# ZhonghuaYi/EI-Nexus_official

Hardware: AMD Instinct MI355X
Metric: event-image pairs/s (extract+match, 346x260, 1024 kpts) (higher is better)
Workload: dtype f32; 1 GPU; B32 346x260 5-bin event voxel + gray image, VGG(event)+SuperPoint(image) extractors, MNN matcher, k=1024; global_batch=32, event_bins=5, parallelism=dp1 (pairs sharded, metric all-reduce only), log_assignment=False, dense_outputs=False, same_scene_pairs=False, weights=seeded synthetic, descriptor-head bias calibrated (per-channel mean removed)

## Files before the change

ei-nexus_official_amd/csrc/detect.hip:

```cpp
#include <algorithm>

#include "einx_common.h"

namespace {

__device__ __forceinline__ bool mask_on(const uint8_t* mask, int b, int H, int W, int h0, int w0, int Hp, int Wp, int y, int x,
                                        int dilate, int replicate) {
  const int r = dilate ? 1 : 0;
  bool any = false;
#pragma unroll
  for (int dy = -1; dy <= 1; ++dy)
#pragma unroll
    for (int dx = -1; dx <= 1; ++dx) {
      const int yy = y + dy, xx = x + dx, sy = yy - h0, sx = xx - w0;
      const bool ok = dy >= -r && dy <= r && dx >= -r && dx <= r && yy >= 0 && yy < Hp && xx >= 0 && xx < Wp &&
                      (replicate || (sy >= 0 && sy < H && sx >= 0 && sx < W));
      const uint8_t m = mask[((size_t)b * H + min(max(sy, 0), H - 1)) * W + min(max(sx, 0), W - 1)];
      any |= ok && m != 0;
    }
  return any;
}

__global__ __launch_bounds__(256) void score65_kernel(const float* logits, int B, int hc, int wc, const uint8_t* mask, int H, int W,
                                                      int h0, int w0, int dilate, int replicate, int border, float* prob, float* score,
                                                      int32_t* zero_ptr, int zero_n, float* crop) {
  if ((int)(blockIdx.x * 256 + threadIdx.x) < zero_n) zero_ptr[blockIdx.x * 256 + threadIdx.x] = 0;
  const int cells = hc * wc;
  const int lane = threadIdx.x & 63, wave = threadIdx.x >> 6;
  const int j = lane & 7, i = lane >> 3;
  const int gid = (blockIdx.x * 4 + wave) * 8 + j;
  const bool valid = gid < B * cells;
  const int g = valid ? gid : B * cells - 1;
  const int b = g / cells, cell = g % cells;
  const int h = cell / wc, w = cell % wc;
  const float* l = logits + (size_t)b * 65 * cells + cell;
  float v[8];
#pragma unroll
  for (int k = 0; k < 8; ++k) v[k] = l[(size_t)(8 * i + k) * cells];
  const float v64 = l[(size_t)64 * cells];
  float mx = v64;
#pragma unroll
  for (int k = 0; k < 8; ++k) mx = fmaxf(mx, v[k]);
  mx = fmaxf(mx, __shfl_xor(mx, 8, 64));
  mx = fmaxf(mx, __shfl_xor(mx, 16, 64));
  mx = fmaxf(mx, __shfl_xor(mx, 32, 64));
  float e[8];
#pragma unroll
  for (int k = 0; k < 8; ++k) e[k] = einx_expf(v[k] - mx);
  const float e64 = einx_expf(v64 - mx);
  float s = 0.0f;
#pragma unroll
  for (int c = 0; c < 64; ++c) s = s + __shfl(e[c & 7], j + 8 * (c >> 3), 64);
  s = s + e64;
  if (!valid) return;
  const int Hp = hc * 8, Wp = wc * 8;
  float* pr = prob + (size_t)b * 65 * cells + cell;
  const int y = h * 8 + i;
  unsigned cols = 0x3ffu;
  if (mask) {
    cols = 0;
    const int r = dilate ? 1 : 0;
#pragma unroll
    for (int dy = -1; dy <= 1; ++dy) {
      const int yy = y + dy, sy = yy - h0;
      const bool rok = dy >= -r && dy <= r && yy >= 0 && yy < Hp && (replicate || (sy >= 0 && sy < H));
      const uint8_t* mrow = mask + ((size_t)b * H + min(max(sy, 0), H - 1)) * W;
      uint8_t m[10];
#pragma unroll
      for (int k = 0; k < 10; ++k) m[k] = mrow[min(max(w * 8 - 1 + k - w0, 0), W - 1)];
#pragma unroll
      for (int k = 0; k < 10; ++k) {
        const int xx = w * 8 - 1 + k, sx = xx - w0;
        if (rok && xx >= 0 && xx < Wp && (replicate || (sx >= 0 && sx < W)) && m[k]) cols |= 1u << k;
      }
    }
  }
  const unsigned window = (mask && !dilate) ? 2u : 7u;
  float out[8];
#pragma unroll
  for (int k = 0; k < 8; ++k) {
    const float p = e[k] / s;
    pr[(size_t)(8 * i + k) * cells] = p;
    const int x = w * 8 + k;
    float t = p;
    if (!((cols >> k) & window)) t = 0.0f;
    if (border > 0 && (y < border || y >= Hp - border || x < border || x >= Wp - border)) t = 0.0f;
    out[k] = t;
  }
  if (i == 0) pr[(size_t)64 * cells] = e64 / s;
  f32x4* dst = reinterpret_cast<f32x4*>(score + ((size_t)b * Hp + y) * Wp + w * 8);
  dst[0] = f32x4{out[0], out[1], out[2], out[3]};
  dst[1] = f32x4{out[4], out[5], out[6], out[7]};
  if (crop) {
    const int uy = y - h0;
    if (uy >= 0 && uy < H) {
      float* cr = crop + ((size_t)b * H + uy) * W - w0 + w * 8;
#pragma unroll
      for (int k = 0; k < 8; ++k) {
        const int ux = w * 8 + k - w0;
        if (ux >= 0 && ux < W) cr[k] = out[k];
      }
    }
  }
}

__global__ void score1_kernel(const float* logits, int B, int Hp, int Wp, const uint8_t* mask, int H, int W, int h0, int w0,
                              int dilate, int replicate, int border, float* prob, float* score, int32_t* zero_ptr, int zero_n,
                              float* crop) {
  const int n = Hp * Wp;
  const int gid = blockIdx.x * blockDim.x + threadIdx.x;
  if (gid < zero_n) zero_ptr[gid] = 0;
  if (gid >= B * n) return;
  const int b = gid / n, p = gid % n;
  const int y = p / Wp, x = p % Wp;
  float v = einx_sigmoidf(logits[gid]);
  if (mask && !mask_on(mask, b, H, W, h0, w0, Hp, Wp, y, x, dilate, replicate)) v = 0.0f;
  if (border > 0 && (y < border || y >= Hp - border || x < border || x >= Wp - border)) v = 0.0f;
  prob[gid] = v;
  score[gid] = v;
  if (crop) {
    const int uy = y - h0, ux = x - w0;
    if (uy >= 0 && uy < H && ux >= 0 && ux < W) crop[((size_t)b * H + uy) * W + ux] = v;
  }
}

__global__ void dense_positions_kernel(const float* score, int B, int H, int W, int xy, float* out) {
  const size_t n = (size_t)B * H * W;
  const size_t gid = (size_t)blockIdx.x * blockDim.x + threadIdx.x;
  if (gid >= n) return;
  const int p = (int)(gid % ((size_t)H * W));
  const float fy = (float)(p / W) + 0.5f, fx = (float)(p % W) + 0.5f;
  float* o = out + gid * 3;
  o[0] = xy ? fx : fy;
  o[1] = xy ? fy : fx;
  o[2] = score[gid];
}

__global__ void border_kernel(float* score, int B, int Hp, int Wp, int border) {
  const int n = Hp * Wp;
  const int gid = blockIdx.x * blockDim.x + threadIdx.x;
  if (gid >= B * n) return;
  const int p = gid % n;
  const int y = p / Wp, x = p % Wp;
  if (y < border || y >= Hp - border || x < border || x >= Wp - border) score[gid] = 0.0f;
}

constexpr int NMS_TH = 32, NMS_TW = 64, NMS_MAXR = 4, NMS_THREADS = 512;

template <int R>
__global__ __launch_bounds__(NMS_THREADS) void nms_pass_kernel(const float* src, float* dst, int Hp, int Wp, int tilesX, int tilesY,
                                                       int32_t* flags, int it, int nIt) {
  constexpr int VH = NMS_TH + 4 * R, VW = NMS_TW + 4 * R;
  constexpr int MH = NMS_TH + 2 * R, MW = NMS_TW + 2 * R;
// ... 42 lines not shown
  for (int i = tid; i < MH * MW; i += NMS_THREADS) {
    const int my = i / MW, mx = i % MW;
    const int vy = my + R;
    const float* row = vals + vy * VW + mx;
    const float c = row[R];
    const int y = y0 - R + my, x = x0 - R + mx;
    float left = row[0], right = row[R + 1];
#pragma unroll
    for (int dx = 1; dx < R; ++dx) {
      left = fmaxf(left, row[dx]);
      right = fmaxf(right, row[R + 1 + dx]);
    }
    float above = r9[(vy - R) * MW + mx], below = r9[(vy + 1) * MW + mx];
#pragma unroll
    for (int dy = 1; dy < R; ++dy) {
      above = fmaxf(above, r9[(vy - R + dy) * MW + mx]);
      below = fmaxf(below, r9[(vy + 1 + dy) * MW + mx]);
    }
    const bool ok = y >= 0 && y < Hp && x >= 0 && x < Wp && left < c && above < c && right <= c && below <= c;
    ismax[i] = ok ? 1 : 0;
  }
  __syncthreads();
  for (int i = tid; i < MH * NMS_TW; i += NMS_THREADS) {
    const int my = i / NMS_TW, tx = i % NMS_TW;
    const uint8_t* row = ismax + my * MW + tx;
    unsigned o = 0;
#pragma unroll
    for (int dx = 0; dx <= 2 * R; ++dx) o |= row[dx];
    rowor[i] = (uint8_t)o;
  }
  __syncthreads();
  int my_changed = 0;
  for (int i = tid; i < NMS_TH * NMS_TW; i += NMS_THREADS) {
    const int ty = i / NMS_TW, tx = i % NMS_TW;
    const int y = y0 + ty, x = x0 + tx;
    if (y >= Hp || x >= Wp) continue;
    const float c = vals[(ty + 2 * R) * VW + tx + 2 * R];
    unsigned o = 0;
#pragma unroll
    for (int dy = 0; dy <= 2 * R; ++dy) o |= rowor[(ty + dy) * NMS_TW + tx];
    const bool sup = o != 0 && !ismax[(ty + R) * MW + tx + R];
    float out = c;
    if (c != 0.0f && sup) {
      out = 0.0f;
      my_changed = 1;
    }
    d[(size_t)y * Wp + x] = out;
  }
  if (my_changed) changed = 1;
  __syncthreads();
  if (tid == 0 && changed) atomicOr(&flags[b * nIt + it], 1);
}

struct __attribute__((aligned(16))) Nms4Smem {
  static constexpr int R = 4;
  static constexpr int VH = NMS_TH + 4 * R, VW = NMS_TW + 4 * R;
  static constexpr int MH = NMS_TH + 2 * R, MW = NMS_TW + 2 * R;
  static constexpr int G = MW / 8, TG = NMS_TW / 8;
  float vals[VH * VW];
  float r9[VH * MW];
  uint8_t rowok8[VH * G];
  uint8_t ismax8[MH * (G + 1)];
  uint8_t rowor8[MH * TG];
  int changed;
};

template <bool COHERENT>
__device__ __forceinline__ void nms4_tile(Nms4Smem& sm, const float* s, float* d, int Hp, int Wp, int y0, int x0) {
  constexpr int R = Nms4Smem::R, VH = Nms4Smem::VH, VW = Nms4Smem::VW, MH = Nms4Smem::MH, MW = Nms4Smem::MW, G = Nms4Smem::G, TG = Nms4Smem::TG;
  const int tid = threadIdx.x;
  constexpr int NLOAD = (VH * VW + NMS_THREADS - 1) / NMS_THREADS;
  float staged[NLOAD];
#pragma unroll
  for (int k = 0; k < NLOAD; ++k) {
    const int i = tid + k * NMS_THREADS;
    const int ii = i < VH * VW ? i : 0;
    const int y = y0 - 2 * R + ii / VW, x = x0 - 2 * R + ii % VW;
    const bool in = y >= 0 && y < Hp && x >= 0 && x < Wp;
    const float* src_p = s + (size_t)(in ? y : 0) * Wp + (in ? x : 0);
    const float v = COHERENT ? __hip_atomic_load(const_cast<float*>(src_p), __ATOMIC_RELAXED, __HIP_MEMORY_SCOPE_AGENT) : *src_p;
    staged[k] = in ? v : 0.0f;
  }
#pragma unroll
  for (int k = 0; k < NLOAD; ++k) {
    const int i = tid + k * NMS_THREADS;
    if (i < VH * VW) sm.vals[i] = staged[k];
  }
  __syncthreads();
  if (tid < VH * G) {
    const int vy = tid / G, g = tid % G;
    float v[16];
    const float* row = sm.vals + vy * VW + g * 8;
#pragma unroll
    for (int q = 0; q < 4; ++q) {
      const f32x4 t = *reinterpret_cast<const f32x4*>(row + 4 * q);
      v[4 * q] = t[0];
      v[4 * q + 1] = t[1];
      v[4 * q + 2] = t[2];
      v[4 * q + 3] = t[3];
    }
    float m9[8];
    unsigned ok = 0;
#pragma unroll
    for (int k = 0; k < 8; ++k) {
      float left = v[k], right = v[k + 5];
#pragma unroll
      for (int t = 1; t < 4; ++t) {
        left = fmaxf(left, v[k + t]);
        right = fmaxf(right, v[k + 5 + t]);
      }
      const float c = v[k + 4];
      m9[k] = fmaxf(fmaxf(left, right), c);
      ok |= (left < c && right <= c) ? (1u << k) : 0u;
    }
    float* o = sm.r9 + vy * MW + g * 8;
    *reinterpret_cast<f32x4*>(o) = f32x4{m9[0], m9[1], m9[2], m9[3]};
    *reinterpret_cast<f32x4*>(o + 4) = f32x4{m9[4], m9[5], m9[6], m9[7]};
    sm.rowok8[tid] = (uint8_t)ok;
  }
  __syncthreads();
  if (tid < MH * G) {
    const int my = tid / G, g = tid % G;
    const int vy = my + R;
    float above[8], below[8];
#pragma unroll
    for (int k = 0; k < 8; ++k) above[k] = below[k] = 0.0f;
#pragma unroll
    for (int dy = 1; dy <= R; ++dy) {
      const float* ra = sm.r9 + (vy - dy) * MW + g * 8;
      const float* rb = sm.r9 + (vy + dy) * MW + g * 8;
      const f32x4 a0 = *reinterpret_cast<const f32x4*>(ra), a1 = *reinterpret_cast<const f32x4*>(ra + 4);
      const f32x4 b0 = *reinterpret_cast<const f32x4*>(rb), b1 = *reinterpret_cast<const f32x4*>(rb + 4);
#pragma unroll
      for (int k = 0; k < 4; ++k) {
        above[k] = dy == 1 ? a0[k] : fmaxf(above[k], a0[k]);
        above[k + 4] = dy == 1 ? a1[k] : fmaxf(above[k + 4], a1[k]);
        below[k] = dy == 1 ? b0[k] : fmaxf(below[k], b0[k]);
        below[k + 4] = dy == 1 ? b1[k] : fmaxf(below[k + 4], b1[k]);
      }
    }
    const float* crow = sm.vals + vy * VW + g * 8 + R;
    const f32x4 c0 = *reinterpret_cast<const f32x4*>(crow), c1 = *reinterpret_cast<const f32x4*>(crow + 4);
    const unsigned rok = sm.rowok8[vy * G + g];
    const int y = y0 - R + my;
    unsigned bits = 0;
#pragma unroll
    for (int k = 0; k < 8; ++k) {
      const float c = k < 4 ? c0[k] : c1[k - 4];
      const int x = x0 - R + g * 8 + k;
      const bool okk = ((rok >> k) & 1u) && y >= 0 && y < Hp && x >= 0 && x < Wp && above[k] < c && below[k] <= c;
      bits |= okk ? (1u << k) : 0u;
    }
    sm.ismax8[my * (G + 1) + g] = (uint8_t)bits;
    if (g == 0) sm.ismax8[my * (G + 1) + G] = 0;
  }
  __syncthreads();
  if (tid < MH * TG) {
    const int my = tid / TG, t8 = tid % TG;
    const unsigned w = (unsigned)sm.ismax8[my * (G + 1) + t8] | ((unsigned)sm.ismax8[my * (G + 1) + t8 + 1] << 8) |
                       ((unsigned)sm.ismax8[my * (G + 1) + t8 + 2] << 16);
    unsigned r = 0;
#pragma unroll
    for (int dx = 0; dx <= 2 * R; ++dx) r |= w >> dx;
    sm.rowor8[tid] = (uint8_t)(r & 0xFFu);
  }
  __syncthreads();
  int my_changed = 0;
  if (tid < NMS_TH * TG) {
    const int ty = tid / TG, t8 = tid % TG;
    unsigned o8 = 0;
#pragma unroll
    for (int dy = 0; dy <= 2 * R; ++dy) o8 |= sm.rowor8[(ty + dy) * TG + t8];
    const unsigned iw = (unsigned)sm.ismax8[(ty + R) * (G + 1) + t8] | ((unsigned)sm.ismax8[(ty + R) * (G + 1) + t8 + 1] << 8);
    const unsigned is8 = (iw >> R) & 0xFFu;
    const unsigned sup = o8 & ~is8;
    const float* crow = sm.vals + (ty + 2 * R) * VW + t8 * 8 + 2 * R;
    const f32x4 c0 = *reinterpret_cast<const f32x4*>(crow), c1 = *reinterpret_cast<const f32x4*>(crow + 4);
    const int y = y0 + ty;
    if (y < Hp) {
      float out[8];
#pragma unroll
      for (int k = 0; k < 8; ++k) {
        const float c = k < 4 ? c0[k] : c1[k - 4];
        const bool kill = c != 0.0f && ((sup >> k) & 1u);
        out[k] = kill ? 0.0f : c;
        if (kill && x0 + t8 * 8 + k < Wp) my_changed = 1;
      }
      float* o = d + (size_t)y * Wp + x0 + t8 * 8;
      if (x0 + t8 * 8 + 7 < Wp && (Wp & 3) == 0) {
        *reinterpret_cast<f32x4*>(o) = f32x4{out[0], out[1], out[2], out[3]};
        *reinterpret_cast<f32x4*>(o + 4) = f32x4{out[4], out[5], out[6], out[7]};
      } else {
#pragma unroll
        for (int k = 0; k < 8; ++k)
          if (x0 + t8 * 8 + k < Wp) o[k] = out[k];
      }
    }
  }
  if (my_changed) sm.changed = 1;
}

__global__ __launch_bounds__(NMS_THREADS) void nms_pass4_kernel(const float* src, float* dst, int Hp, int Wp, int tilesX, int tilesY,
                                                                int32_t* flags, int it, int nIt) {
  __shared__ Nms4Smem sm;
  int bid = xcd_contiguous((int)blockIdx.x, (int)gridDim.x);
  const int txi = bid % tilesX;
  bid /= tilesX;
  const int tyi = bid % tilesY;
  const int b = bid / tilesY;
  if (it >= 2 && flags[b * nIt + it - 1] == 0) return;
  if (threadIdx.x == 0) sm.changed = 0;
  nms4_tile<false>(sm, src + (size_t)b * Hp * Wp, dst + (size_t)b * Hp * Wp, Hp, Wp, tyi * NMS_TH, txi * NMS_TW);
  __syncthreads();
  if (threadIdx.x == 0 && sm.changed) atomicOr(&flags[b * nIt + it], 1);
}

constexpr int NMS_FIN_MAXT = 2048;
constexpr int kNmsFinishMaxPasses = 256;
__global__ __launch_bounds__(NMS_THREADS) void nms4_finish_kernel(float* bufA, float* bufB, int Hp, int Wp, int tilesX, int tilesY,
                                                                  int32_t* flags, int nIt, int max_passes) {
  __shared__ Nms4Smem sm;
  __shared__ uint8_t dirty[2][NMS_FIN_MAXT];
  __shared__ int any_changed;
  const int b = blockIdx.x;
  if (flags[b * nIt + nIt - 1] == 0) return;
  const int tid = threadIdx.x;
  const int ntiles = tilesX * tilesY;
  const bool track = ntiles <= NMS_FIN_MAXT;
  float* src = bufA + (size_t)b * Hp * Wp;
  float* dst = bufB + (size_t)b * Hp * Wp;
  if (track)
    for (int i = tid; i < ntiles; i += NMS_THREADS) {
      dirty[0][i] = 1;
      dirty[1][i] = 0;
    }
  __syncthreads();
  int cur = 0;
  int left = 1;
  for (int pass = 0; pass < max_passes; ++pass) {
    if (tid == 0) any_changed = 0;
    for (int t = 0; t < ntiles; ++t) {
      const int txi = t % tilesX, tyi = t / tilesX;
      bool need = !track;
      if (track) {
        for (int dy = -1; dy <= 1 && !need; ++dy)
          for (int dx = -1; dx <= 1; ++dx) {
            const int yy = tyi + dy, xx = txi + dx;
            if (yy >= 0 && yy < tilesY && xx >= 0 && xx < tilesX && dirty[cur][yy * tilesX + xx]) need = true;
          }
      }
      if (!need) continue;
      if (tid == 0) sm.changed = 0;
      __syncthreads();
      nms4_tile<true>(sm, src, dst, Hp, Wp, tyi * NMS_TH, txi * NMS_TW);
      __syncthreads();
      if (tid == 0 && sm.changed) {
        any_changed = 1;
        if (track) dirty[cur ^ 1][t] = 1;
      }
      __syncthreads();
    }
    asm volatile("s_waitcnt vmcnt(0)" ::: "memory");
    __syncthreads();
    left = any_changed;
    if (track)
      for (int i = tid; i < ntiles; i += NMS_THREADS) dirty[cur][i] = 0;
    cur ^= 1;
    float* tmp = src;
    src = dst;
    dst = tmp;
    __syncthreads();
    if (!left) break;
  }
  if (tid == 0) flags[b * nIt + nIt - 1] = left ? 1 : 0;
}

constexpr int SEL_THREADS = 1024;

struct SelArgs {
  const float* map;
  const int32_t* flags;
  float* nms_out;
  float* positions;
  int32_t* indices;
  int32_t* counts;
  float* thr_out;
  int32_t* not_converged;
  int Hp, Wp, H, W, h0, w0;
  int top_k, lo, hi, cap, ordering_xy, nIt;
  float det_thr;
};

__device__ __forceinline__ int block_excl_scan(int v, int* total, int* scratch ) {
  const int lane = threadIdx.x & 63, wave = threadIdx.x >> 6;
  int incl = v;
#pragma unroll
  for (int off = 1; off < 64; off <<= 1) {
    const int t = __shfl_up(incl, off, 64);
    if (lane >= off) incl += t;
  }
  if (lane == 63) scratch[wave] = incl;
  __syncthreads();
  if (threadIdx.x == 0) {
    int run = 0;
    for (int w = 0; w < SEL_THREADS / 64; ++w) {
      const int t = scratch[w];
      scratch[w] = run;
// ... 328 lines not shown
    if (i < nz) {
      v = cval[i];
      fi = cidx[i];
      y = fi / a.Wp;
      x = fi % a.Wp;
      const int uy = y - a.h0, ux = x - a.w0;
      keep = v > thr && uy >= 0 && uy < a.H && ux >= 0 && ux < a.W;
    }
    int total;
    const int pos = base + block_excl_scan(keep ? 1 : 0, &total, scratch);
    if (keep && pos < a.cap) {
      const float py = ((float)y + 0.5f) - (float)a.h0, px = ((float)x + 0.5f) - (float)a.w0;
      float* o = a.positions + ((size_t)b * a.cap + pos) * 3;
      o[0] = a.ordering_xy ? px : py;
      o[1] = a.ordering_xy ? py : px;
      o[2] = v;
      a.indices[(size_t)b * a.cap + pos] = fi;
    }
    base += total;
  }
  if (tid == 0) a.counts[b] = base;
}

__global__ void nms_crop_kernel(const float* map, const float* thr, int B, int Hp, int Wp, int h0, int w0, int H, int W, float* out) {
  const size_t n = (size_t)B * H * W;
  const size_t gid = (size_t)blockIdx.x * blockDim.x + threadIdx.x;
  if (gid >= n) return;
  const int b = (int)(gid / ((size_t)H * W));
  const int r = (int)(gid % ((size_t)H * W));
  const float v = map[((size_t)b * Hp + (r / W + h0)) * Wp + r % W + w0];
  out[gid] = v > thr[b] ? v : 0.0f;
}

void topk_ranks(int N, int k, int* lo, int* hi) {
  const float q = (float)(N - k) / (float)N;
  const float rank = q * (float)(N - 1);
  *lo = (int)floorf(rank);
  *hi = (int)ceilf(rank);
}

}

EINX_EXPORT int einx_score_map(const float* logits, int B, int C, int hc, int wc, const uint8_t* mask, int H, int W, int h0, int w0,
                               int dilate, int border, float* prob, float* score, void* stream) {
  return einx_score_map_zero(logits, B, C, hc, wc, mask, H, W, h0, w0, dilate, EINX_MASK_PAD_ZERO, border, prob, score, nullptr, 0, nullptr,
                             stream);
}

EINX_EXPORT int einx_score_map_pad(const float* logits, int B, int C, int hc, int wc, const uint8_t* mask, int mask_pad, int H, int W, int h0,
                                   int w0, int dilate, int border, float* prob, float* score, void* stream) {
  return einx_score_map_zero(logits, B, C, hc, wc, mask, H, W, h0, w0, dilate, mask_pad, border, prob, score, nullptr, 0, nullptr, stream);
}

int einx_score_map_zero(const float* logits, int B, int C, int hc, int wc, const uint8_t* mask, int H, int W, int h0, int w0, int dilate,
                        int mask_pad, int border, float* prob, float* score, int32_t* zero_ptr, int zero_n, float* crop, void* stream) {
  EINX_CHECK_ARG(mask_pad == EINX_MASK_PAD_ZERO || mask_pad == EINX_MASK_PAD_REPLICATE, "mask_pad must be EINX_MASK_PAD_ZERO or EINX_MASK_PAD_REPLICATE");
  EINX_CHECK_ARG(!mask || (H > 0 && W > 0), "a mask needs the un-padded size");
  const int replicate = mask_pad == EINX_MASK_PAD_REPLICATE;
  EINX_CHECK_ARG(!crop || (H > 0 && W > 0), "the cropped map needs the un-padded size");
  EINX_CHECK_ARG(logits && prob && score, "null pointer");
  EINX_CHECK_ARG(zero_n == 0 || (zero_ptr && (long)zero_n <= (long)(C == 65 ? einx_cdiv(B * hc * wc, 32) : einx_cdiv(B * hc * wc, 256)) * 256),
                 "more words to zero than threads in the launch");
  EINX_CHECK_ARG(C == 65 || C == 1, "detector head must have 65 or 1 channels");
  EINX_CHECK_ARG(B > 0 && hc > 0 && wc > 0, "bad shape");
  hipStream_t s = (hipStream_t)stream;
  EINX_PROF("score_map (score65/score1)", s);
  if (C == 65) {
    const int n = B * hc * wc;
    hipLaunchKernelGGL(score65_kernel, dim3(einx_cdiv(n, 32)), dim3(256), 0, s, logits, B, hc, wc, mask, H, W, h0, w0, dilate, replicate, border,
                       prob, score, zero_ptr, zero_n, crop);
  } else {
    const int n = B * hc * wc;
    hipLaunchKernelGGL(score1_kernel, dim3(einx_cdiv(n, 256)), dim3(256), 0, s, logits, B, hc, wc, mask, H, W, h0, w0, dilate, replicate, border,
                       prob, score, zero_ptr, zero_n, crop);
  }
  EINX_CHECK_LAUNCH();
  return EINX_OK;
}

EINX_EXPORT int einx_remove_border(float* score, int B, int Hp, int Wp, int border, void* stream) {
  EINX_CHECK_ARG(score, "null pointer");
  if (border <= 0) return EINX_OK;
  const int n = B * Hp * Wp;
  hipLaunchKernelGGL(border_kernel, dim3(einx_cdiv(n, 256)), dim3(256), 0, (hipStream_t)stream, score, B, Hp, Wp, border);
  EINX_CHECK_LAUNCH();
  return EINX_OK;
}

EINX_EXPORT int einx_dense_positions(const float* score, int B, int H, int W, int ordering_xy, float* out, void* stream) {
  EINX_CHECK_ARG(score && out, "null pointer");
  EINX_CHECK_ARG(B > 0 && H > 0 && W > 0, "bad shape");
  const size_t n = (size_t)B * H * W;
  hipLaunchKernelGGL(dense_positions_kernel, dim3((unsigned)((n + 255) / 256)), dim3(256), 0, (hipStream_t)stream, score, B, H, W, ordering_xy, out);
  EINX_CHECK_LAUNCH();
  return EINX_OK;
}

EinxDetectWs einx_detect_carve(WsCarver& c, const einx_detect_params* p) {
  const size_t map = (size_t)p->B * p->Hp * p->Wp;
  const EinxDetectWs w{c.take<float>(map), c.take<float>(map), c.take<int32_t>((size_t)p->B * (p->nms_iters > 0 ? p->nms_iters : 1)),
                       p->radius > 0 ? p->B * p->nms_iters : 0};
  c.slack(256);
  return w;
}

EINX_EXPORT size_t einx_detect_ws_bytes(const einx_detect_params* p) {
  if (!p) return 0;
  WsCarver c{nullptr};
  einx_detect_carve(c, p);
  return c.bytes;
}

EINX_EXPORT int einx_detect(const float* score, const einx_detect_params* p, void* ws, float* nms_out, float* positions,
                            int32_t* indices, int32_t* counts, float* thr, int32_t* not_converged, void* stream) {
  return einx_detect_prezeroed(score, p, ws, nms_out, positions, indices, counts, thr, not_converged, 0, nullptr, stream);
}

int einx_detect_prezeroed(const float* score, const einx_detect_params* p, void* ws, float* nms_out, float* positions, int32_t* indices,
                          int32_t* counts, float* thr, int32_t* not_converged, int flags_zeroed, const float** final_map, void* stream) {
  EINX_CHECK_ARG(score && p && ws && positions && indices && counts && thr && not_converged, "null pointer");
  EINX_CHECK_ARG(p->B > 0 && p->Hp > 0 && p->Wp > 0 && p->cap > 0, "bad shape");
  EINX_CHECK_ARG(p->radius >= 0 && p->radius <= NMS_MAXR, "nms radius must be in 0..4");
  EINX_CHECK_ARG(p->radius == 0 || p->nms_iters >= 1, "nms_iters must be >= 1");
  EINX_CHECK_ARG((size_t)p->Hp * p->Wp < (1u << 30), "map too large");
  hipStream_t s = (hipStream_t)stream;
  const int N = p->Hp * p->Wp;
  WsCarver c{(char*)ws};
  const auto [buf0, buf1, flags, nflags] = einx_detect_carve(c, p);
  const float* cur = score;
  const int nIt = p->radius > 0 ? p->nms_iters : 0;
  if (nIt > 0) {
    if (!flags_zeroed && hipMemsetAsync(flags, 0, (size_t)nflags * sizeof(int32_t), s) != hipSuccess) {
      einx_set_error("einx_detect: memset failed");
      return EINX_ERR_LAUNCH;
    }
    const int tilesX = einx_cdiv(p->Wp, NMS_TW), tilesY = einx_cdiv(p->Hp, NMS_TH);
    const dim3 grid((unsigned)(tilesX * tilesY * p->B));
    for (int it = 0; it < nIt; ++it) {
      float* dst = (it & 1) ? buf1 : buf0;
      EINX_PROF("nms_pass", s);
      switch (p->radius) {
        case 1: hipLaunchKernelGGL(nms_pass_kernel<1>, grid, dim3(NMS_THREADS), 0, s, cur, dst, p->Hp, p->Wp, tilesX, tilesY, flags, it, nIt); break;
        case 2: hipLaunchKernelGGL(nms_pass_kernel<2>, grid, dim3(NMS_THREADS), 0, s, cur, dst, p->Hp, p->Wp, tilesX, tilesY, flags, it, nIt); break;
        case 3: hipLaunchKernelGGL(nms_pass_kernel<3>, grid, dim3(NMS_THREADS), 0, s, cur, dst, p->Hp, p->Wp, tilesX, tilesY, flags, it, nIt); break;
        default: hipLaunchKernelGGL(nms_pass4_kernel, grid, dim3(NMS_THREADS), 0, s, cur, dst, p->Hp, p->Wp, tilesX, tilesY, flags, it, nIt); break;
      }
      EINX_CHECK_LAUNCH();
      cur = dst;
    }
    if (p->radius == 4) {
      float* last = const_cast<float*>(cur);
      float* other = last == buf0 ? buf1 : buf0;
      EINX_PROF("nms4_finish_kernel", s);
      hipLaunchKernelGGL(nms4_finish_kernel, dim3((unsigned)p->B), dim3(NMS_THREADS), 0, s, last, other, p->Hp, p->Wp, tilesX, tilesY, flags, nIt,
                         std::max(kNmsFinishMaxPasses, p->Hp + p->Wp));
      EINX_CHECK_LAUNCH();
    }
  }
  SelArgs a;
  a.map = cur;
  a.flags = flags;
  a.nms_out = nullptr;
  a.positions = positions;
  a.indices = indices;
  a.counts = counts;
  a.thr_out = thr;
  a.not_converged = not_converged;
  a.Hp = p->Hp;
  a.Wp = p->Wp;
  a.H = p->H;
  a.W = p->W;
  a.h0 = p->h0;
  a.w0 = p->w0;
  a.top_k = p->top_k;
  a.cap = p->cap;
  a.ordering_xy = p->ordering_xy;
  a.nIt = nIt;
  a.det_thr = p->det_thr;
  a.lo = a.hi = 0;
  if (p->top_k > 0 && p->top_k < N) topk_ranks(N, p->top_k, &a.lo, &a.hi);
  {
    EINX_PROF("select_compact_kernel", s);
    hipLaunchKernelGGL(select_compact_kernel, dim3(p->B), dim3(SEL_THREADS), 0, s, a);
  }
  if (final_map) *final_map = a.map;
  if (nms_out && !final_map) {
    EINX_PROF("nms_crop_kernel", s);
    EINX_CHECK_LAUNCH();
    const size_t n = (size_t)p->B * p->H * p->W;
    hipLaunchKernelGGL(nms_crop_kernel, dim3((unsigned)((n + 255) / 256)), dim3(256), 0, s, a.map, thr, p->B, p->Hp, p->Wp, p->h0, p->w0, p->H, p->W,
                       nms_out);
  }
  EINX_CHECK_LAUNCH();
  return EINX_OK;
}
```

ei-nexus_official_amd/csrc/einx_common.h:

```cpp
#pragma once
#include <hip/hip_runtime.h>
#include <stdint.h>

#include <mutex>

#include "../../include/einx.h"
#include "../../include/einx_math.h"

#define EINX_EXPORT extern "C" __attribute__((visibility("default")))


void einx_set_error(const char* fmt, ...);

#define EINX_CHECK_ARG(cond, msg)                 \
  do {                                            \
    if (!(cond)) {                                \
      einx_set_error("%s: %s", __func__, msg);    \
      return EINX_ERR_ARG;                        \
    }                                             \
  } while (0)

#define EINX_CHECK_LAUNCH()                                                   \
  do {                                                                        \
    hipError_t e_ = hipGetLastError();                                        \
// ... 45 lines not shown

struct EinxWatch {
  const int64_t* table;
  const unsigned long long* ref;
  unsigned long long* hash;
  int32_t* flag;
  int n, bit;
};
#ifdef __HIPCC__
__device__ __forceinline__ unsigned long long einx_watch_term(unsigned long long pos, uint32_t word) {
  const unsigned long long coef = (2ull * pos + 1ull) * 0x9E3779B97F4A7C15ull;
  const unsigned long long t = ((unsigned long long)word + 1ull) * coef;
  return t ^ (t >> 29);
}
__device__ __forceinline__ void einx_watch_tensor(const EinxWatch& w, int t, int lane) {
  const uint32_t* p = reinterpret_cast<const uint32_t*>((uintptr_t)w.table[2 * t]);
  const long long n = w.table[2 * t + 1];
  unsigned long long h = 0;
  long long i0 = 0;
  if ((((uintptr_t)p) & 15) == 0) {
    typedef uint32_t u32x4 __attribute__((ext_vector_type(4)));
    const u32x4* p4 = reinterpret_cast<const u32x4*>(p);
    const long long n4 = n >> 2;
    for (long long j0 = 0; j0 < n4; j0 += 64 * 8) {
      u32x4 v[8];
#pragma unroll
      for (int u = 0; u < 8; ++u) {
        const long long j = j0 + lane + 64 * u;
        v[u] = p4[j < n4 ? j : n4 - 1];
      }
#pragma unroll
      for (int u = 0; u < 8; ++u) {
        const long long j = j0 + lane + 64 * u;
        if (j < n4) {
#pragma unroll
          for (int e = 0; e < 4; ++e) h += einx_watch_term((unsigned long long)(4 * j + e), v[u][e]);
        }
      }
    }
    i0 = n4 << 2;
  }
  for (long long i = i0 + lane; i < n; i += 64) h += einx_watch_term((unsigned long long)i, p[i]);
#pragma unroll
  for (int off = 32; off >= 1; off >>= 1) h += __shfl_xor(h, off, 64);
  if (lane == 0) {
    if (w.ref) {
      if (w.ref[t] != h) atomicOr(w.flag, w.bit);
    } else {
      w.hash[t] = h;
    }
  }
}
#endif
int einx_score_map_zero(const float* logits, int B, int C, int hc, int wc, const uint8_t* mask, int H, int W, int h0, int w0, int dilate,
                        int mask_pad, int border, float* prob, float* score, int32_t* zero_ptr, int zero_n, float* crop, void* stream);
struct EinxDetectWs {
  float *buf0, *buf1;
  int32_t* flags;
  int nflags;
};
EinxDetectWs einx_detect_carve(WsCarver& c, const einx_detect_params* p);
int einx_detect_prezeroed(const float* score, const einx_detect_params* p, void* ws, float* nms_out, float* positions, int32_t* indices,
                          int32_t* counts, float* thr, int32_t* not_converged, int flags_zeroed, const float** final_map, void* stream);
struct EinxCrop {
  const float* map;
  const float* thr;
  float* out;
  int Hp, Wp, h0, w0, H, W;
};
#ifdef __HIPCC__
__device__ __forceinline__ void einx_crop_block(const EinxCrop& c, int b, int blk, int tid) {
  const int r = blk * 256 + tid;
  if (r >= c.H * c.W) return;
  const float v = c.map[((size_t)b * c.Hp + (r / c.W + c.h0)) * c.Wp + r % c.W + c.w0];
  c.out[(size_t)b * c.H * c.W + r] = v > c.thr[b] ? v : 0.0f;
}
#endif
int einx_desc_sample_watch(const float* raw, int B, int D, int hc, int wc, int Hp, int Wp, int bilinear, int channels_last, const int32_t* indices,
                           const int32_t* counts, int cap, float scale, float* out, const EinxWatch& watch, const EinxCrop& crop, void* stream);

typedef float f32x16 __attribute__((ext_vector_type(16)));
typedef float f32x4 __attribute__((ext_vector_type(4)));

static inline __host__ __device__ int einx_cdiv(int a, int b) { return (a + b - 1) / b; }
```

ei-nexus_official_amd/csrc/extract.hip:

```cpp
#include <stdlib.h>
#include <string.h>

#include <algorithm>
#include <mutex>
#include <new>
#include <vector>

#include "einx_common.h"

struct einx_extractor {
  einx_extractor_desc d;
  std::vector<einx_conv_desc> backbone, det, desc;
  bool has_merged = false;
  einx_conv_desc merged;
  std::vector<einx_conv_desc_f16> backbone16, det16, desc16;
  einx_conv_desc_f16 merged16 = {};
};

namespace {

struct Plan {
  int Hp, Wp, h0, w0;
  int hc, wc;
  size_t buf_elems[2];
// ... 276 lines not shown
    }
    cur = out;
  }
  auto run_head = [&](const std::vector<einx_conv_desc>& L, const std::vector<einx_conv_desc_f16>& L16, float* scratch, float* final_out, void* st) -> int {
    const float* x = o->feats;
    for (size_t i = 0; i < L.size(); ++i) {
      float* out = (i + 1 < L.size()) ? scratch : final_out;
      const int r = conv(x, h, w, &L[i], f16_of(L16, i), out, st);
      if (r) return r;
      x = out;
    }
    return 0;
  };
  const int D = e->desc.back().cout;
  const bool merged = e->has_merged && B == 1;
  if (merged && (rc = conv(o->feats, h, w, &e->merged, &e->merged16, wk.head, stream))) return rc;
  const float* desc_in = wk.head + (size_t)e->det.front().cout * h * w;
  auto det_branch = [&](void* st) -> int {
    if (merged) return conv(wk.head, h, w, &e->det[1], f16_of(e->det16, 1), o->logits, st);
    return run_head(e->det, e->det16, wk.head, o->logits, st);
  };
  auto desc_branch = [&](void* st) -> int {
    int r = merged ? conv(desc_in, h, w, &e->desc[1], f16_of(e->desc16, 1), o->raw, st) : run_head(e->desc, e->desc16, head2, o->raw, st);
    if (r) return r;
    if (e->d.cell == 8) r = einx_normalize_map(o->raw, B, D, h * w, e->d.desc_scale, o->coarse, o->raw_cl, st);
    return r;
  };
  std::unique_lock<std::mutex> side_lock;
  const EinxSide* sd = fork ? einx_side_acquire((hipStream_t)stream, &side_lock) : nullptr;
  if (sd) {
    if (hipEventRecord(sd->fork, (hipStream_t)stream) != hipSuccess || hipStreamWaitEvent(sd->stream, sd->fork, 0) != hipSuccess) {
      einx_set_error("einx_extract: fork failed");
      return EINX_ERR_LAUNCH;
    }
    rc = desc_branch(sd->stream);
    const bool ok = hipEventRecord(sd->join, sd->stream) == hipSuccess;
    if (rc) {
      (void)hipStreamWaitEvent((hipStream_t)stream, sd->join, 0);
      return rc;
    }
    if (!ok) {
      einx_set_error("einx_extract: join failed");
      return EINX_ERR_LAUNCH;
    }
    if ((rc = det_branch(stream))) {
      (void)hipStreamWaitEvent((hipStream_t)stream, sd->join, 0);
      return rc;
    }
  } else {
    if ((rc = det_branch(stream))) return rc;
    if ((rc = desc_branch(stream))) return rc;
  }
  const int C_det = e->det.back().cout;
  const long score_threads = (long)(C_det == 65 ? einx_cdiv(B * h * w, 32) : einx_cdiv(B * h * w, 256)) * 256;
  const bool zero_in_score = wk.det.nflags > 0 && wk.det.nflags <= score_threads;
  rc = einx_score_map_zero(o->logits, B, C_det, h, w, mask, H, W, pl.h0, pl.w0, e->d.dilate_mask, mask_pad, e->d.border, o->prob, o->score,
                           zero_in_score ? wk.det.flags : nullptr, zero_in_score ? wk.det.nflags : 0, o->score_crop, stream);
  if (rc) {
    if (sd) (void)hipStreamWaitEvent((hipStream_t)stream, sd->join, 0);
    return rc;
  }
  const float* nms_map = nullptr;
  rc = einx_detect_prezeroed(o->score, &dp, wk.det_ws, o->nms, o->positions, o->indices, o->counts, o->thr, o->not_converged, zero_in_score ? 1 : 0,
                             o->nms ? &nms_map : nullptr, stream);
  if (sd && hipStreamWaitEvent((hipStream_t)stream, sd->join, 0) != hipSuccess && !rc) {
    einx_set_error("einx_extract: join failed");
    return EINX_ERR_LAUNCH;
  }
  if (rc) return rc;
  const bool bilinear = e->d.cell == 8;
  const bool use_cl = bilinear && D <= 512;
  EinxWatch watch;
  const bool on = ww && ww->n > 0;
  watch.table = on ? ww->table : nullptr;
  watch.ref = on ? (const unsigned long long*)ww->ref : nullptr;
  watch.hash = on ? (unsigned long long*)ww->scratch : nullptr;
  watch.flag = on ? ww->stale : nullptr;
  watch.n = on ? ww->n : 0;
  watch.bit = 1;
  EinxCrop crop{};
  crop.map = o->nms ? nms_map : nullptr;
  crop.thr = o->thr;
  crop.out = o->nms;
  crop.Hp = pl.Hp;
  crop.Wp = pl.Wp;
  crop.h0 = pl.h0;
  crop.w0 = pl.w0;
  crop.H = H;
  crop.W = W;
  return einx_desc_sample_watch(use_cl ? o->raw_cl : o->raw, B, D, h, w, pl.Hp, pl.Wp, bilinear ? 1 : 0, use_cl ? 1 : 0, o->indices, o->counts,
                                o->cap, e->d.desc_scale, o->sparse_desc, watch, crop, stream);
}
```

Before: 3754 pairs/s.

## Stage score65 outputs in LDS, add region-masked NMS wakeups and vector loads

The score65 kernel now assigns one block per cell row chunk. It stages the mask window, the softmax probabilities and the score tiles in shared memory so that the global stores for prob, score and crop are coalesced, replacing the strided per-cell writes. NMS pass flags now carry per-region bits, so later iterations and the finish kernel only revisit tiles next to regions that changed, not the whole image. Non-coherent NMS tile loads use 16-byte vector reads when aligned, and asm barriers are added to shape register scheduling. The cost is more shared memory, extra block barriers and a 32-region cap on the flag granularity.

```diff
diff --git a/ei-nexus_official_amd/csrc/detect.hip b/ei-nexus_official_amd/csrc/detect.hip
--- a/ei-nexus_official_amd/csrc/detect.hip
+++ b/ei-nexus_official_amd/csrc/detect.hip
@@ -21,23 +21,69 @@
   return any;
 }
 
-__global__ __launch_bounds__(256) void score65_kernel(const float* logits, int B, int hc, int wc, const uint8_t* mask, int H, int W,
-                                                      int h0, int w0, int dilate, int replicate, int border, float* prob, float* score,
-                                                      int32_t* zero_ptr, int zero_n, float* crop) {
-  if ((int)(blockIdx.x * 256 + threadIdx.x) < zero_n) zero_ptr[blockIdx.x * 256 + threadIdx.x] = 0;
-  const int cells = hc * wc;
-  const int lane = threadIdx.x & 63, wave = threadIdx.x >> 6;
+constexpr int SC_MAXWAVES = 8, SC_SLOTS = SC_MAXWAVES * 8;
+constexpr int SC_LD = SC_SLOTS + 1;
+constexpr int SC_ROW = SC_SLOTS * 8;
+constexpr int SC_MW = SC_SLOTS * 8 + 8;
+
+inline void score65_geometry(int wc, int* nwaves, int* chunks) {
+  *chunks = einx_cdiv(wc, SC_SLOTS);
+  *nwaves = einx_cdiv(einx_cdiv(wc, *chunks), 8);
+}
+
+__global__ __launch_bounds__(64 * SC_MAXWAVES) void score65_kernel(const float* logits, int B, int hc, int wc, int chunks, const uint8_t* mask,
+                                                                   int H, int W, int h0, int w0, int dilate, int replicate, int border,
+                                                                   float* prob, float* score, int32_t* zero_ptr, int zero_n, float* crop) {
+  __shared__ float pt[65 * SC_LD];
+  __shared__ __attribute__((aligned(16))) float st[8 * SC_ROW];
+  __shared__ __attribute__((aligned(8))) uint8_t mk[10 * SC_MW];
+  const int T = blockDim.x, tid = threadIdx.x;
+  if ((int)(blockIdx.x * T + tid) < zero_n) zero_ptr[blockIdx.x * T + tid] = 0;
+  const int slots = T >> 3;
+  int bid = blockIdx.x;
+  const int ch = bid % chunks;
+  bid /= chunks;
+  const int h = bid % hc, b = bid / hc;
+  const int wbase = ch * slots;
+  const int nc = min(slots, wc - wbase);
+  const int cells = hc * wc, Hp = hc * 8, Wp = wc * 8;
+  const size_t cell0 = (size_t)b * 65 * cells + (size_t)h * wc + wbase;
+  const int jc = tid % slots, c0 = tid / slots;
+  if (mask) {
+    const int cw = 8 * nc + 2;
+    const int lane = tid & 63, nw = T >> 6;
+    for (int ry = tid >> 6; ry < 10; ry += nw) {
+      const int yy = 8 * h - 1 + ry, sy = yy - h0;
+      const bool rok = yy >= 0 && yy < Hp && (replicate || (sy >= 0 && sy < H));
+      const uint8_t* mrow = mask + ((size_t)b * H + min(max(sy, 0), H - 1)) * W;
+      constexpr int NU = (SC_SLOTS * 8 + 2 + 63) / 64;
+      uint8_t m[NU];
+#pragma unroll
+      for (int u = 0; u < NU; ++u) {
+        const int cx = lane + 64 * u;
+        m[u] = 0;
+        if (cx < cw) m[u] = mrow[min(max(8 * wbase - 1 + cx - w0, 0), W - 1)];
+      }
+#pragma unroll
+      for (int u = 0; u < NU; ++u) {
+        const int cx = lane + 64 * u;
+        const int xx = 8 * wbase - 1 + cx, sx = xx - w0;
+        const bool cok = xx >= 0 && xx < Wp && (replicate || (sx >= 0 && sx < W));
+        if (cx < cw) mk[ry * SC_MW + cx] = (cok && rok && m[u]) ? 1 : 0;
+      }
+    }
+  }
+  __syncthreads();
+  const int lane = tid & 63, wave = tid >> 6;
   const int j = lane & 7, i = lane >> 3;
-  const int gid = (blockIdx.x * 4 + wave) * 8 + j;
-  const bool valid = gid < B * cells;
-  const int g = valid ? gid : B * cells - 1;
-  const int b = g / cells, cell = g % cells;
-  const int h = cell / wc, w = cell % wc;
-  const float* l = logits + (size_t)b * 65 * cells + cell;
+  const int js = wave * 8 + j;
+  const bool valid = js < nc;
+  const int w = wbase + js;
   float v[8];
-#pragma unroll
-  for (int k = 0; k < 8; ++k) v[k] = l[(size_t)(8 * i + k) * cells];
-  const float v64 = l[(size_t)64 * cells];
+  const float* lcell = logits + cell0 + min(js, nc - 1);
+#pragma unroll
+  for (int k = 0; k < 8; ++k) v[k] = lcell[(8 * i + k) * cells];
+  const float v64 = lcell[64 * cells];
   float mx = v64;
 #pragma unroll
   for (int k = 0; k < 8; ++k) mx = fmaxf(mx, v[k]);
@@ -50,55 +96,76 @@
   const float e64 = einx_expf(v64 - mx);
   float s = 0.0f;
 #pragma unroll
-  for (int c = 0; c < 64; ++c) s = s + __shfl(e[c & 7], j + 8 * (c >> 3), 64);
+  for (int c = 0; c < 64; ++c) {
+    if (c > 0 && (c & 15) == 0) {
+#pragma unroll
+      for (int k = 0; k < 8; ++k) asm volatile("" : "+v"(e[k]) : "v"(s));
+    }
+    s = s + __shfl(e[c & 7], j + 8 * (c >> 3), 64);
+  }
   s = s + e64;
-  if (!valid) return;
-  const int Hp = hc * 8, Wp = wc * 8;
-  float* pr = prob + (size_t)b * 65 * cells + cell;
   const int y = h * 8 + i;
   unsigned cols = 0x3ffu;
   if (mask) {
+    unsigned long long lo = 0;
+    unsigned hi = 0;
+    const int r = dilate ? 1 : 0;
+#pragma unroll
+    for (int dy = -1; dy <= 1; ++dy) {
+      const uint8_t* row = mk + (i + 1 + dy) * SC_MW + 8 * js;
+      const unsigned long long a = *reinterpret_cast<const unsigned long long*>(row);
+      const unsigned c2 = *reinterpret_cast<const unsigned*>(row + 8);
+      if (dy >= -r && dy <= r) {
+        lo |= a;
+        hi |= c2;
+      }
+    }
     cols = 0;
-    const int r = dilate ? 1 : 0;
-#pragma unroll
-    for (int dy = -1; dy <= 1; ++dy) {
-      const int yy = y + dy, sy = yy - h0;
-      const bool rok = dy >= -r && dy <= r && yy >= 0 && yy < Hp && (replicate || (sy >= 0 && sy < H));
-      const uint8_t* mrow = mask + ((size_t)b * H + min(max(sy, 0), H - 1)) * W;
-      uint8_t m[10];
-#pragma unroll
-      for (int k = 0; k < 10; ++k) m[k] = mrow[min(max(w * 8 - 1 + k - w0, 0), W - 1)];
-#pragma unroll
-      for (int k = 0; k < 10; ++k) {
-        const int xx = w * 8 - 1 + k, sx = xx - w0;
-        if (rok && xx >= 0 && xx < Wp && (replicate || (sx >= 0 && sx < W)) && m[k]) cols |= 1u << k;
-      }
-    }
+#pragma unroll
+    for (int k = 0; k < 8; ++k) cols |= (unsigned)((lo >> (8 * k)) & 1ull) << k;
+    cols |= (hi & 1u) << 8;
+    cols |= ((hi >> 8) & 1u) << 9;
   }
   const unsigned window = (mask && !dilate) ? 2u : 7u;
   float out[8];
 #pragma unroll
   for (int k = 0; k < 8; ++k) {
     const float p = e[k] / s;
-    pr[(size_t)(8 * i + k) * cells] = p;
+    if (valid) pt[(8 * i + k) * SC_LD + js] = p;
     const int x = w * 8 + k;
     float t = p;
     if (!((cols >> k) & window)) t = 0.0f;
     if (border > 0 && (y < border || y >= Hp - border || x < border || x >= Wp - border)) t = 0.0f;
     out[k] = t;
   }
-  if (i == 0) pr[(size_t)64 * cells] = e64 / s;
-  f32x4* dst = reinterpret_cast<f32x4*>(score + ((size_t)b * Hp + y) * Wp + w * 8);
-  dst[0] = f32x4{out[0], out[1], out[2], out[3]};
-  dst[1] = f32x4{out[4], out[5], out[6], out[7]};
+  if (valid && i == 0) pt[64 * SC_LD + js] = e64 / s;
+  f32x4* so = reinterpret_cast<f32x4*>(st + i * SC_ROW + 8 * js);
+  so[0] = f32x4{out[0], out[1], out[2], out[3]};
+  so[1] = f32x4{out[4], out[5], out[6], out[7]};
+  __syncthreads();
+#pragma unroll
+  for (int r = 0; r < 9; ++r) {
+    const int c = c0 + 8 * r;
+    if (c < 65 && jc < nc) prob[cell0 + (c * cells + jc)] = pt[c * SC_LD + jc];
+  }
+  {
+    const int qs = T >> 2;
+    const int m = tid % qs, row0 = tid / qs;
+    if (m < 2 * nc) {
+#pragma unroll
+      for (int r = 0; r < 2; ++r) {
+        const int row = row0 + 4 * r;
+        *reinterpret_cast<f32x4*>(score + ((size_t)b * Hp + 8 * h + row) * Wp + 8 * wbase + 4 * m) = *reinterpret_cast<const f32x4*>(st + row * SC_ROW + 4 * m);
+      }
+    }
+  }
   if (crop) {
-    const int uy = y - h0;
-    if (uy >= 0 && uy < H) {
-      float* cr = crop + ((size_t)b * H + uy) * W - w0 + w * 8;
-#pragma unroll
-      for (int k = 0; k < 8; ++k) {
-        const int ux = w * 8 + k - w0;
-        if (ux >= 0 && ux < W) cr[k] = out[k];
+    const int ux = 8 * wbase + tid - w0;
+    if (tid < 8 * nc && ux >= 0 && ux < W) {
+#pragma unroll
+      for (int row = 0; row < 8; ++row) {
+        const int uy = 8 * h + row - h0;
+        if (uy >= 0 && uy < H) crop[((size_t)b * H + uy) * W + ux] = st[row * SC_ROW + tid];
       }
     }
   }
@@ -247,6 +314,30 @@
   if (tid == 0 && changed) atomicOr(&flags[b * nIt + it], 1);
 }
 
+struct NmsRegions {
+  int sx, sy, nx;
+};
+
+NmsRegions nms_regions(int tilesX, int tilesY) {
+  int sx = 1, sy = 1;
+  while (einx_cdiv(tilesX, sx) * einx_cdiv(tilesY, sy) > 32) {
+    if (einx_cdiv(tilesX, sx) >= einx_cdiv(tilesY, sy)) ++sx;
+    else ++sy;
+  }
+  return NmsRegions{sx, sy, einx_cdiv(tilesX, sx)};
+}
+
+__device__ __forceinline__ unsigned nms_region_bit(const NmsRegions& g, int txi, int tyi) { return 1u << ((tyi / g.sy) * g.nx + txi / g.sx); }
+
+__device__ __forceinline__ unsigned nms_wake_mask(const NmsRegions& g, int txi, int tyi, int tilesX, int tilesY) {
+  const int rx0 = max(txi - 1, 0) / g.sx, rx1 = min(txi + 1, tilesX - 1) / g.sx;
+  const int ry0 = max(tyi - 1, 0) / g.sy, ry1 = min(tyi + 1, tilesY - 1) / g.sy;
+  unsigned m = 0;
+  for (int ry = ry0; ry <= ry1; ++ry)
+    for (int rx = rx0; rx <= rx1; ++rx) m |= 1u << (ry * g.nx + rx);
+  return m;
+}
+
 struct __attribute__((aligned(16))) Nms4Smem {
   static constexpr int R = 4;
   static constexpr int VH = NMS_TH + 4 * R, VW = NMS_TW + 4 * R;
@@ -261,25 +352,44 @@
 };
 
 template <bool COHERENT>
-__device__ __forceinline__ void nms4_tile(Nms4Smem& sm, const float* s, float* d, int Hp, int Wp, int y0, int x0) {
+__device__ __forceinline__ void nms4_tile(Nms4Smem& sm, const float* s, float* d, int Hp, int Wp, int y0, int x0, bool vec16) {
   constexpr int R = Nms4Smem::R, VH = Nms4Smem::VH, VW = Nms4Smem::VW, MH = Nms4Smem::MH, MW = Nms4Smem::MW, G = Nms4Smem::G, TG = Nms4Smem::TG;
   const int tid = threadIdx.x;
-  constexpr int NLOAD = (VH * VW + NMS_THREADS - 1) / NMS_THREADS;
-  float staged[NLOAD];
-#pragma unroll
-  for (int k = 0; k < NLOAD; ++k) {
-    const int i = tid + k * NMS_THREADS;
-    const int ii = i < VH * VW ? i : 0;
-    const int y = y0 - 2 * R + ii / VW, x = x0 - 2 * R + ii % VW;
-    const bool in = y >= 0 && y < Hp && x >= 0 && x < Wp;
-    const float* src_p = s + (size_t)(in ? y : 0) * Wp + (in ? x : 0);
-    const float v = COHERENT ? __hip_atomic_load(const_cast<float*>(src_p), __ATOMIC_RELAXED, __HIP_MEMORY_SCOPE_AGENT) : *src_p;
-    staged[k] = in ? v : 0.0f;
-  }
-#pragma unroll
-  for (int k = 0; k < NLOAD; ++k) {
-    const int i = tid + k * NMS_THREADS;
-    if (i < VH * VW) sm.vals[i] = staged[k];
+  if (!COHERENT && vec16) {
+    constexpr int VG = VW / 4, NG = VH * VG, NLOAD4 = (NG + NMS_THREADS - 1) / NMS_THREADS;
+    f32x4 staged[NLOAD4];
+#pragma unroll
+    for (int k = 0; k < NLOAD4; ++k) {
+      const int i = tid + k * NMS_THREADS;
+      const int ii = i < NG ? i : 0;
+      const int y = y0 - 2 * R + ii / VG, x = x0 - 2 * R + 4 * (ii % VG);
+      const bool in = y >= 0 && y < Hp && x >= 0 && x < Wp;
+      const f32x4 v = *reinterpret_cast<const f32x4*>(s + (size_t)(in ? y : 0) * Wp + (in ? x : 0));
+      staged[k] = in ? v : f32x4{0.0f, 0.0f, 0.0f, 0.0f};
+    }
+#pragma unroll
+    for (int k = 0; k < NLOAD4; ++k) {
+      const int i = tid + k * NMS_THREADS;
+      if (i < NG) *reinterpret_cast<f32x4*>(sm.vals + 4 * i) = staged[k];
+    }
+  } else {
+    constexpr int NLOAD = (VH * VW + NMS_THREADS - 1) / NMS_THREADS;
+    float staged[NLOAD];
+#pragma unroll
+    for (int k = 0; k < NLOAD; ++k) {
+      const int i = tid + k * NMS_THREADS;
+      const int ii = i < VH * VW ? i : 0;
+      const int y = y0 - 2 * R + ii / VW, x = x0 - 2 * R + ii % VW;
+      const bool in = y >= 0 && y < Hp && x >= 0 && x < Wp;
+      const float* src_p = s + (size_t)(in ? y : 0) * Wp + (in ? x : 0);
+      const float v = COHERENT ? __hip_atomic_load(const_cast<float*>(src_p), __ATOMIC_RELAXED, __HIP_MEMORY_SCOPE_AGENT) : *src_p;
+      staged[k] = in ? v : 0.0f;
+    }
+#pragma unroll
+    for (int k = 0; k < NLOAD; ++k) {
+      const int i = tid + k * NMS_THREADS;
+      if (i < VH * VW) sm.vals[i] = staged[k];
+    }
   }
   __syncthreads();
   if (tid < VH * G) {
@@ -320,10 +430,12 @@
     float above[8], below[8];
 #pragma unroll
     for (int k = 0; k < 8; ++k) above[k] = below[k] = 0.0f;
+    int vyr = vy;
 #pragma unroll
     for (int dy = 1; dy <= R; ++dy) {
-      const float* ra = sm.r9 + (vy - dy) * MW + g * 8;
-      const float* rb = sm.r9 + (vy + dy) * MW + g * 8;
+      if (dy == 3) asm volatile("" : "+v"(vyr) : "v"(above[0]), "v"(above[1]), "v"(above[2]), "v"(above[3]), "v"(above[4]), "v"(above[5]), "v"(above[6]), "v"(above[7]), "v"(below[0]), "v"(below[1]), "v"(below[2]), "v"(below[3]), "v"(below[4]), "v"(below[5]), "v"(below[6]), "v"(below[7]));
+      const float* ra = sm.r9 + (vyr - dy) * MW + g * 8;
+      const float* rb = sm.r9 + (vyr + dy) * MW + g * 8;
       const f32x4 a0 = *reinterpret_cast<const f32x4*>(ra), a1 = *reinterpret_cast<const f32x4*>(ra + 4);
       const f32x4 b0 = *reinterpret_cast<const f32x4*>(rb), b1 = *reinterpret_cast<const f32x4*>(rb + 4);
 #pragma unroll
@@ -396,29 +508,34 @@
 }
 
 __global__ __launch_bounds__(NMS_THREADS) void nms_pass4_kernel(const float* src, float* dst, int Hp, int Wp, int tilesX, int tilesY,
-                                                                int32_t* flags, int it, int nIt) {
+                                                                int32_t* flags, int it, int nIt, NmsRegions g) {
   __shared__ Nms4Smem sm;
   int bid = xcd_contiguous((int)blockIdx.x, (int)gridDim.x);
   const int txi = bid % tilesX;
   bid /= tilesX;
   const int tyi = bid % tilesY;
   const int b = bid / tilesY;
-  if (it >= 2 && flags[b * nIt + it - 1] == 0) return;
+  if (it >= 2) {
+    const unsigned prev = (unsigned)flags[b * nIt + it - 1];
+    if (prev == 0 || (prev & nms_wake_mask(g, txi, tyi, tilesX, tilesY)) == 0) return;
+  }
   if (threadIdx.x == 0) sm.changed = 0;
-  nms4_tile<false>(sm, src + (size_t)b * Hp * Wp, dst + (size_t)b * Hp * Wp, Hp, Wp, tyi * NMS_TH, txi * NMS_TW);
-  __syncthreads();
-  if (threadIdx.x == 0 && sm.changed) atomicOr(&flags[b * nIt + it], 1);
+  const bool vec16 = (Wp & 3) == 0 && (reinterpret_cast<size_t>(src) & 15) == 0;
+  nms4_tile<false>(sm, src + (size_t)b * Hp * Wp, dst + (size_t)b * Hp * Wp, Hp, Wp, tyi * NMS_TH, txi * NMS_TW, vec16);
+  __syncthreads();
+  if (threadIdx.x == 0 && sm.changed) atomicOr(reinterpret_cast<unsigned*>(&flags[b * nIt + it]), nms_region_bit(g, txi, tyi));
 }
 
 constexpr int NMS_FIN_MAXT = 2048;
 constexpr int kNmsFinishMaxPasses = 256;
 __global__ __launch_bounds__(NMS_THREADS) void nms4_finish_kernel(float* bufA, float* bufB, int Hp, int Wp, int tilesX, int tilesY,
-                                                                  int32_t* flags, int nIt, int max_passes) {
+                                                                  int32_t* flags, int nIt, int max_passes, NmsRegions g) {
   __shared__ Nms4Smem sm;
   __shared__ uint8_t dirty[2][NMS_FIN_MAXT];
   __shared__ int any_changed;
   const int b = blockIdx.x;
-  if (flags[b * nIt + nIt - 1] == 0) return;
+  const unsigned last_changed = (unsigned)flags[b * nIt + nIt - 1];
+  if (last_changed == 0) return;
   const int tid = threadIdx.x;
   const int ntiles = tilesX * tilesY;
   const bool track = ntiles <= NMS_FIN_MAXT;
@@ -426,7 +543,7 @@
   float* dst = bufB + (size_t)b * Hp * Wp;
   if (track)
     for (int i = tid; i < ntiles; i += NMS_THREADS) {
-      dirty[0][i] = 1;
+      dirty[0][i] = nIt < 2 || (last_changed & nms_region_bit(g, i % tilesX, i / tilesX)) ? 1 : 0;
       dirty[1][i] = 0;
     }
   __syncthreads();
@@ -447,7 +564,7 @@
       if (!need) continue;
       if (tid == 0) sm.changed = 0;
       __syncthreads();
-      nms4_tile<true>(sm, src, dst, Hp, Wp, tyi * NMS_TH, txi * NMS_TW);
+      nms4_tile<true>(sm, src, dst, Hp, Wp, tyi * NMS_TH, txi * NMS_TW, false);
       __syncthreads();
       if (tid == 0 && sm.changed) {
         any_changed = 1;
@@ -882,6 +999,13 @@
   return einx_score_map_zero(logits, B, C, hc, wc, mask, H, W, h0, w0, dilate, mask_pad, border, prob, score, nullptr, 0, nullptr, stream);
 }
 
+long einx_score_map_threads(int B, int C, int hc, int wc) {
+  if (C != 65) return (long)einx_cdiv(B * hc * wc, 256) * 256;
+  int nwaves, chunks;
+  score65_geometry(wc, &nwaves, &chunks);
+  return (long)B * hc * chunks * 64 * nwaves;
+}
+
 int einx_score_map_zero(const float* logits, int B, int C, int hc, int wc, const uint8_t* mask, int H, int W, int h0, int w0, int dilate,
                         int mask_pad, int border, float* prob, float* score, int32_t* zero_ptr, int zero_n, float* crop, void* stream) {
   EINX_CHECK_ARG(mask_pad == EINX_MASK_PAD_ZERO || mask_pad == EINX_MASK_PAD_REPLICATE, "mask_pad must be EINX_MASK_PAD_ZERO or EINX_MASK_PAD_REPLICATE");
@@ -889,16 +1013,17 @@
   const int replicate = mask_pad == EINX_MASK_PAD_REPLICATE;
   EINX_CHECK_ARG(!crop || (H > 0 && W > 0), "the cropped map needs the un-padded size");
   EINX_CHECK_ARG(logits && prob && score, "null pointer");
-  EINX_CHECK_ARG(zero_n == 0 || (zero_ptr && (long)zero_n <= (long)(C == 65 ? einx_cdiv(B * hc * wc, 32) : einx_cdiv(B * hc * wc, 256)) * 256),
-                 "more words to zero than threads in the launch");
   EINX_CHECK_ARG(C == 65 || C == 1, "detector head must have 65 or 1 channels");
   EINX_CHECK_ARG(B > 0 && hc > 0 && wc > 0, "bad shape");
+  EINX_CHECK_ARG((long)hc * wc * 64 * C < (1L << 31), "map too large");
+  EINX_CHECK_ARG(zero_n == 0 || (zero_ptr && (long)zero_n <= einx_score_map_threads(B, C, hc, wc)), "more words to zero than threads in the launch");
   hipStream_t s = (hipStream_t)stream;
   EINX_PROF("score_map (score65/score1)", s);
   if (C == 65) {
-    const int n = B * hc * wc;
-    hipLaunchKernelGGL(score65_kernel, dim3(einx_cdiv(n, 32)), dim3(256), 0, s, logits, B, hc, wc, mask, H, W, h0, w0, dilate, replicate, border,
-                       prob, score, zero_ptr, zero_n, crop);
+    int nwaves, chunks;
+    score65_geometry(wc, &nwaves, &chunks);
+    hipLaunchKernelGGL(score65_kernel, dim3((unsigned)(B * hc * chunks)), dim3(64 * nwaves), 0, s, logits, B, hc, wc, chunks, mask, H, W, h0, w0, dilate,
+                       replicate, border, prob, score, zero_ptr, zero_n, crop);
   } else {
     const int n = B * hc * wc;
     hipLaunchKernelGGL(score1_kernel, dim3(einx_cdiv(n, 256)), dim3(256), 0, s, logits, B, hc, wc, mask, H, W, h0, w0, dilate, replicate, border,
@@ -966,6 +1091,7 @@
     }
     const int tilesX = einx_cdiv(p->Wp, NMS_TW), tilesY = einx_cdiv(p->Hp, NMS_TH);
     const dim3 grid((unsigned)(tilesX * tilesY * p->B));
+    const NmsRegions regions = nms_regions(tilesX, tilesY);
     for (int it = 0; it < nIt; ++it) {
       float* dst = (it & 1) ? buf1 : buf0;
       EINX_PROF("nms_pass", s);
@@ -973,7 +1099,7 @@
         case 1: hipLaunchKernelGGL(nms_pass_kernel<1>, grid, dim3(NMS_THREADS), 0, s, cur, dst, p->Hp, p->Wp, tilesX, tilesY, flags, it, nIt); break;
         case 2: hipLaunchKernelGGL(nms_pass_kernel<2>, grid, dim3(NMS_THREADS), 0, s, cur, dst, p->Hp, p->Wp, tilesX, tilesY, flags, it, nIt); break;
         case 3: hipLaunchKernelGGL(nms_pass_kernel<3>, grid, dim3(NMS_THREADS), 0, s, cur, dst, p->Hp, p->Wp, tilesX, tilesY, flags, it, nIt); break;
-        default: hipLaunchKernelGGL(nms_pass4_kernel, grid, dim3(NMS_THREADS), 0, s, cur, dst, p->Hp, p->Wp, tilesX, tilesY, flags, it, nIt); break;
+        default: hipLaunchKernelGGL(nms_pass4_kernel, grid, dim3(NMS_THREADS), 0, s, cur, dst, p->Hp, p->Wp, tilesX, tilesY, flags, it, nIt, regions); break;
       }
       EINX_CHECK_LAUNCH();
       cur = dst;
@@ -983,7 +1109,7 @@
       float* other = last == buf0 ? buf1 : buf0;
       EINX_PROF("nms4_finish_kernel", s);
       hipLaunchKernelGGL(nms4_finish_kernel, dim3((unsigned)p->B), dim3(NMS_THREADS), 0, s, last, other, p->Hp, p->Wp, tilesX, tilesY, flags, nIt,
-                         std::max(kNmsFinishMaxPasses, p->Hp + p->Wp));
+                         std::max(kNmsFinishMaxPasses, p->Hp + p->Wp), regions);
       EINX_CHECK_LAUNCH();
     }
   }
diff --git a/ei-nexus_official_amd/csrc/einx_common.h b/ei-nexus_official_amd/csrc/einx_common.h
--- a/ei-nexus_official_amd/csrc/einx_common.h
+++ b/ei-nexus_official_amd/csrc/einx_common.h
@@ -121,6 +121,7 @@
   }
 }
 #endif
+long einx_score_map_threads(int B, int C, int hc, int wc);
 int einx_score_map_zero(const float* logits, int B, int C, int hc, int wc, const uint8_t* mask, int H, int W, int h0, int w0, int dilate,
                         int mask_pad, int border, float* prob, float* score, int32_t* zero_ptr, int zero_n, float* crop, void* stream);
 struct EinxDetectWs {
diff --git a/ei-nexus_official_amd/csrc/extract.hip b/ei-nexus_official_amd/csrc/extract.hip
--- a/ei-nexus_official_amd/csrc/extract.hip
+++ b/ei-nexus_official_amd/csrc/extract.hip
@@ -352,7 +352,7 @@
     if ((rc = desc_branch(stream))) return rc;
   }
   const int C_det = e->det.back().cout;
-  const long score_threads = (long)(C_det == 65 ? einx_cdiv(B * h * w, 32) : einx_cdiv(B * h * w, 256)) * 256;
+  const long score_threads = einx_score_map_threads(B, C_det, h, w);
   const bool zero_in_score = wk.det.nflags > 0 && wk.det.nflags <= score_threads;
   rc = einx_score_map_zero(o->logits, B, C_det, h, w, mask, H, W, pl.h0, pl.w0, e->d.dilate_mask, mask_pad, e->d.border, o->prob, o->score,
                            zero_in_score ? wk.det.flags : nullptr, zero_in_score ? wk.det.nflags : 0, o->score_crop, stream);
```

Result: no change. 3777 pairs/s (median of 3 runs) (+0.6%).
